# wenbowen123/catgrasp

Measured on NVIDIA H100. Metric: candidate grasps scored/sec, higher is better.
Workload: dtype f32 (128->1024 layer f16 x f16 single pass on wgmma, f32 accumulate; other layers bf16 hi/lo x3)

## Files before the change

catgrasp_b200/csrc/cg_trunk_tc.cu:

```cuda
#include <limits.h>
#include <stdlib.h>

#include <algorithm>

#include "cg_tc_ptx.cuh"
#include "cg_trunk_common.cuh"

namespace {
using namespace cg_trunk;
using namespace cg_ptx;

constexpr int NCW = 8;
constexpr int PROD_WARP = NCW;
constexpr int HELP_WARP = NCW + 1;
constexpr int NHELP = 3 * 32;
constexpr int NTC = (NCW + 4) * 32;
constexpr int NCHUNK = 8;
constexpr uint32_t PIECE = 16384;
__host__ __device__ constexpr int tile_points(int passes) { return passes == 1 ? 256 : 128; }
constexpr uint32_t W1_OFF = 0;
constexpr uint32_t W2_OFF = PIECE;
constexpr uint32_t X3_OFF = 3 * PIECE;
constexpr uint32_t X3_BYTES = 4 * PIECE;
constexpr uint32_t RING_OFF = X3_OFF + X3_BYTES;
constexpr uint32_t RING_BYTES = 6 * PIECE;
constexpr uint32_t KEYS_OFF = RING_OFF + RING_BYTES;
constexpr uint32_t KEYS_BYTES = 2 * 1024 * 4;
constexpr uint32_t MISC_OFF = KEYS_OFF + KEYS_BYTES;
constexpr int NSLOT_MAX = 6;
constexpr uint32_t IMG_W3B = NCHUNK * 2 * 2 * PIECE;
constexpr uint32_t IMG_W2 = 2 * PIECE, IMG_W1 = PIECE;
constexpr uint32_t IMG_W2_OFF = IMG_W3B, IMG_W1_OFF = IMG_W3B + IMG_W2;
constexpr uint32_t IMG_W3H_OFF = IMG_W1_OFF + IMG_W1;
constexpr uint32_t IMG_W3H = NCHUNK * 2 * PIECE;

struct Misc {
  float w0[6 * 64];
  float bias0[64];
  float bias1[64];
  float bias2[128];
  double pinv[12];
  double mean[6];
  double sden[6];
  float T3[12];
  unsigned long long full_bar[NSLOT_MAX];
  unsigned long long empty_bar[NSLOT_MAX];
  unsigned long long w_bar;
  unsigned long long cand_bar;
  unsigned long long front_bar;
  unsigned long long keys_bar[2];
};

constexpr size_t SMEM_BYTES = MISC_OFF + sizeof(Misc);
static_assert(SMEM_BYTES <= 232448, "exceeds the 227 KB per-CTA shared memory of sm_90");

#ifdef CG_EXPERIMENTS
enum { TL_START, TL_INPUT, TL_FRONT, TL_X3, TL_L3, TL_L3_WAIT, TL_RING, TL_NPHASE };
constexpr int TL_CTAS = 8, TL_REC = TL_NPHASE + 2;
__host__ __device__ constexpr int TL_STRIDE(int B) { return B >= TL_CTAS ? B / TL_CTAS : 1; }
#define TL_PARAM , unsigned long long *tl
#define TL_ARG(p) , p
#else
#define TL_PARAM
#define TL_ARG(p)
#endif

template <int PASSES>
__global__ void __launch_bounds__(NTC, 1) trunk_tc_kernel(const cg_trunk_args a TL_PARAM) {
  constexpr int TILE = tile_points(PASSES);
  constexpr int NBLK = TILE / 128;
  constexpr int NSLOT = PASSES == 3 ? 3 : 6;
  constexpr uint32_t SLOT_BYTES = PASSES == 3 ? 2 * PIECE : PIECE;
  static_assert(NSLOT * SLOT_BYTES == RING_BYTES, "ring");
  constexpr bool F16 = PASSES < 3;
  constexpr uint32_t X3_KB = TILE * 128;
  constexpr uint32_t X3_LO = 2 * X3_KB;
  static_assert((PASSES == 1 ? 2 : 4) * X3_KB == X3_BYTES, "X3 image");
  extern __shared__ __align__(1024) unsigned char smem[];
  if ((smem_u32(smem) & 1023u) != 0u) __trap();
  Misc &S = *reinterpret_cast<Misc *>(smem + MISC_OFF);
  uint32_t *keys = reinterpret_cast<uint32_t *>(smem + KEYS_OFF);
  const int tid = threadIdx.x, warp = __shfl_sync(0xffffffffu, tid >> 5, 0), lane = tid & 31;
  const int N = a.N;
  const int ntiles = (N + TILE - 1) / TILE;
  const long long T = (long long)a.B * ntiles;
  const int t_begin = (int)(blockIdx.x * T / gridDim.x);
  const int my_tiles = (int)((blockIdx.x + 1) * T / gridDim.x) - t_begin;
  const int b_first = t_begin / ntiles;
  const int ncand = (t_begin + my_tiles - 1) / ntiles - b_first + 1;
  const unsigned char *img = static_cast<const unsigned char *>(a.tc_img);
  const bool has_l1 = a.stage1_mode != 0;
  const uint32_t smem_s = smem_u32(smem);
  const uint32_t w1_s = smem_s + W1_OFF, w2_s = smem_s + W2_OFF, x3_s = smem_s + X3_OFF, ring_s = smem_s + RING_OFF;
  const uint32_t misc_s = smem_s + MISC_OFF;
  const uint32_t full_s = misc_s + (uint32_t)offsetof(Misc, full_bar), empty_s = misc_s + (uint32_t)offsetof(Misc, empty_bar);
  const uint32_t wbar_s = misc_s + (uint32_t)offsetof(Misc, w_bar);
  const uint32_t cand_s = misc_s + (uint32_t)offsetof(Misc, cand_bar), front_s = misc_s + (uint32_t)offsetof(Misc, front_bar);
  const uint32_t keys_s = misc_s + (uint32_t)offsetof(Misc, keys_bar);

  for (int i = tid; i < 6 * 64; i += NTC) S.w0[i] = a.l0.Wt[i];
  if (tid < 64) {
    S.bias0[tid] = a.l0.b[tid];
    S.bias1[tid] = (a.stage1_mode == 1) ? a.l1.b[tid] : 0.f;
  }
  if (tid < 128) S.bias2[tid] = a.l2.b[tid];
  if (a.in.x_direct == nullptr && tid < 6) {
    S.mean[tid] = a.in.mean ? a.in.mean[tid] : 0.0;
    S.sden[tid] = a.in.stdv ? 1.0 / (a.in.stdv[tid] + 1e-15) : 1.0;
  }
  if (tid == 0) {
    for (int i = 0; i < NSLOT; i++) {
      mbar_init(full_s + 8u * i, 1);
      mbar_init(empty_s + 8u * i, NCW);
    }
    mbar_init(wbar_s, 1);
    mbar_init(cand_s, NHELP);
    mbar_init(front_s, NCW * 32);
    mbar_init(keys_s, NCW * 32);
    mbar_init(keys_s + 8u, NCW * 32);
    mbar_init_fence();
  }
  __syncthreads();

  if (warp == PROD_WARP) {
    if (lane == 0) {
      mbar_expect_tx(wbar_s, IMG_W2 + (a.stage1_mode == 1 ? IMG_W1 : 0u));
      bulk_g2s(w2_s, img + IMG_W2_OFF, IMG_W2, wbar_s);
      if (a.stage1_mode == 1) bulk_g2s(w1_s, img + IMG_W1_OFF, IMG_W1, wbar_s);
      const unsigned char *w3src = img + (PASSES == 3 ? 0u : IMG_W3H_OFF);
      const int total = my_tiles * NCHUNK * 2;
      for (int gs = 0; gs < total; gs++) {
        const int s = gs % NSLOT;
        mbar_wait(empty_s + 8u * s, (((uint32_t)(gs / NSLOT)) & 1u) ^ 1u);
        mbar_expect_tx(full_s + 8u * s, SLOT_BYTES);
        bulk_g2s(ring_s + (uint32_t)s * SLOT_BYTES, w3src + (size_t)(gs % (NCHUNK * 2)) * SLOT_BYTES, SLOT_BYTES,
                 full_s + 8u * s);
      }
    }
    return;
  }

  if (warp >= HELP_WARP) {
    const int ht = tid - HELP_WARP * 32;
    for (int k = 0; k <= ncand; k++) {
      if (k < ncand) {
        const int b = b_first + k;
        constexpr int TU = (64 * 8 + NHELP - 1) / NHELP;
        uint32_t t64h[TU][4], t64l[TU][4];
        if (a.stage1_mode == 2) {
          const float *Tb = a.T64 + (size_t)b * 4096;
#pragma unroll
          for (int i = 0; i < TU; i++) {
            const int u = ht + NHELP * i;
            if (u < 512) {
              float v[8];
#pragma unroll
              for (int e = 0; e < 8; e++) v[e] = __ldg(Tb + (8 * (u >> 6) + e) * 64 + (u & 63));
#pragma unroll
              for (int e = 0; e < 4; e++) split_bf16x2(v[2 * e], v[2 * e + 1], t64h[i][e], t64l[i][e]);
            }
          }
        }
        double pinv[12];
        const bool do_pinv = a.in.x_direct == nullptr && ht == 0;
        if (do_pinv) pose_inverse(a.in.poses + (size_t)b * 16, pinv);
        const float t3 = (a.T3 && ht < 9) ? a.T3[b * 9 + ht] : 0.f;
        if (k > 0) mbar_wait(front_s, (uint32_t)(k - 1) & 1u);
        if (a.stage1_mode == 2) {
#pragma unroll
          for (int i = 0; i < TU; i++) {
            const int u = ht + NHELP * i;
            if (u < 512) {
              const uint32_t off = row_chunk_off(u & 63, u >> 6);
              *reinterpret_cast<uint4 *>(smem + W1_OFF + off) =
                  make_uint4(t64h[i][0], t64h[i][1], t64h[i][2], t64h[i][3]);
              *reinterpret_cast<uint4 *>(smem + W1_OFF + 8192 + off) =
                  make_uint4(t64l[i][0], t64l[i][1], t64l[i][2], t64l[i][3]);
            }
          }
          fence_proxy_async();
        }
        if (do_pinv) {
#pragma unroll
          for (int i = 0; i < 12; i++) S.pinv[i] = pinv[i];
        }
        if (ht < 9) S.T3[ht] = t3;
        mbar_arrive(cand_s);
      }
      if (k > 0) {
        const int kp = k - 1;
        mbar_wait(keys_s + 8u * (kp & 1), ((uint32_t)kp >> 1) & 1u);
        const uint32_t *kb = keys + (kp & 1) * 1024;
        uint32_t *g = a.gmax_keys + (size_t)(b_first + kp) * 1024;
        for (int ch = ht; ch < 1024; ch += NHELP) {
          float m = cg_key2f(kb[ch]) + __ldg(&a.l3.b[ch]);
          if (a.relu3) m = fmaxf(m, 0.f);
          atomicMax(&g[ch], cg_f2key(m));
        }
      }
    }
    return;
  }

  const int wg = warp >> 2, w4 = warp & 3, g = lane >> 2, q = lane & 3;
  float vmax = 0.f;
#ifdef CG_EXPERIMENTS
  const bool tl_on = tl != nullptr && blockIdx.x % TL_STRIDE(gridDim.x) == 0 &&
                     (int)(blockIdx.x / TL_STRIDE(gridDim.x)) < TL_CTAS;
  unsigned long long tl_sum[TL_NPHASE] = {}, tl_t0 = clock64(), tl_t = tl_t0, tl_s;
#define TL_MARK(phase)                   \
  do {                                   \
    const unsigned long long _t = clock64(); \
    tl_sum[phase] += _t - tl_t;          \
    tl_t = _t;                           \
  } while (0)
#define TL_SPAN_BEGIN() (tl_s = clock64())
#define TL_SPAN_END(phase) (tl_sum[phase] += clock64() - tl_s)
#else
#define TL_MARK(phase) ((void)0)
#define TL_SPAN_BEGIN() ((void)0)
#define TL_SPAN_END(phase) ((void)0)
#endif
  mbar_wait(wbar_s, 0u);

  auto fetch_id = [&](int b, int n) -> int {
    if (n >= N) n = N - 1;
    return (a.in.x_direct == nullptr && a.in.ids) ? __ldg(a.in.ids + (size_t)b * N + n) : n;
  };
  auto fetch_row = [&](int b, int id, double *r) {
    if (a.in.x_direct) {
      const float *xr = a.in.x_direct + ((size_t)b * N + id) * 6;
#pragma unroll
      for (int k = 0; k < 6; k++) r[k] = __ldg(xr + k);
    } else {
      const double *px = a.in.cloud_xyz + (size_t)id * 3;
      const double *pn = a.in.cloud_nrm + (size_t)id * 3;
#pragma unroll
      for (int k = 0; k < 3; k++) {
        r[k] = __ldg(px + k);
        r[3 + k] = __ldg(pn + k);
      }
    }
  };
  auto finish_row = [&](const double *r, float *v) {
    if (a.in.x_direct) {
#pragma unroll
      for (int k = 0; k < 6; k++) v[k] = (float)r[k];
    } else {
      const double x = r[0], y = r[1], z = r[2];
      const double nx = r[3], ny = r[4], nz = r[5];
      const double *R = S.pinv;
      double w[6];
      w[0] = R[0] * x + R[1] * y + R[2] * z + R[9];
      w[1] = R[3] * x + R[4] * y + R[5] * z + R[10];
      w[2] = R[6] * x + R[7] * y + R[8] * z + R[11];
      w[3] = R[0] * nx + R[1] * ny + R[2] * nz;
      w[4] = R[3] * nx + R[4] * ny + R[5] * nz;
      w[5] = R[6] * nx + R[7] * ny + R[8] * nz;
#pragma unroll
      for (int k = 0; k < 6; k++) v[k] = (float)((w[k] - S.mean[k]) * S.sden[k]);
    }
    if (a.T3) {
      const float x = v[0], y = v[1], z = v[2];
      v[0] = fmaf(z, S.T3[6], fmaf(y, S.T3[3], x * S.T3[0]));
      v[1] = fmaf(z, S.T3[7], fmaf(y, S.T3[4], x * S.T3[1]));
      v[2] = fmaf(z, S.T3[8], fmaf(y, S.T3[5], x * S.T3[2]));
    }
  };

  uint32_t gslot = 0;
  auto slot_of = [&](int c, int kb) { return (gslot + 2u * c + kb) % NSLOT; };
  auto phase_of = [&](int c, int kb) { return ((gslot + 2u * c + kb) / NSLOT) & 1u; };

  auto prow = [&](int blk) { return wg * (TILE / 2) + blk * 64 + w4 * 16 + g; };
  int ids[NBLK][2];
  {
    const int j = t_begin - b_first * ntiles;
#pragma unroll
    for (int blk = 0; blk < NBLK; blk++)
#pragma unroll
      for (int r = 0; r < 2; r++) ids[blk][r] = fetch_id(b_first, j * TILE + prow(blk) + 8 * r);
  }
  TL_MARK(TL_START);
  for (int it = 0; it < my_tiles; it++) {
    const int b = (t_begin + it) / ntiles, j = t_begin + it - b * ntiles, ci = b - b_first;
    const bool cand_first = it == 0 || j == 0, cand_last = it + 1 == my_tiles || j + 1 == ntiles;
    if (cand_first) mbar_wait(cand_s, (uint32_t)ci & 1u);
#pragma unroll 1
    for (int blk = 0; blk < NBLK; blk++) {
      const int p0 = j * TILE + prow(blk);
      float d64[32];
      {
        double r0[6], r1[6];
        fetch_row(b, blk == 0 ? ids[0][0] : ids[NBLK - 1][0], r0);
        fetch_row(b, blk == 0 ? ids[0][1] : ids[NBLK - 1][1], r1);
        float v0[6], v1[6];
        finish_row(r0, v0);
        finish_row(r1, v1);
        TL_MARK(TL_INPUT);
#pragma unroll
        for (int m = 0; m < 8; m++)
#pragma unroll
          for (int e = 0; e < 2; e++) {
            const int c = 8 * m + 2 * q + e;
            float o0 = S.bias0[c], o1 = o0;
#pragma unroll
            for (int k = 0; k < 6; k++) {
              const float w = S.w0[k * 64 + c];
              o0 = fmaf(v0[k], w, o0);
              o1 = fmaf(v1[k], w, o1);
            }
            d64[4 * m + e] = fmaxf(o0, 0.f);
            d64[4 * m + 2 + e] = fmaxf(o1, 0.f);
          }
      }
      uint32_t xh[4][4], xl[4][4];
      if (has_l1) {
        d_to_a<4, false>(d64, xh, xl);
        wg_fence_regs<16>(xh[0]);
        wg_fence_regs<16>(xl[0]);
        wg_fence_regs<32>(d64);
        wg_fence();
#pragma unroll
        for (int ks = 0; ks < 4; ks++) {
          const uint64_t bh = wg_desc(w1_s + 32u * ks), bl = wg_desc(w1_s + 8192u + 32u * ks);
          wg_m64n64<false>(d64, xl[ks], bh, ks > 0 ? 1u : 0u);
          wg_m64n64<false>(d64, xh[ks], bl, 1u);
          wg_m64n64<false>(d64, xh[ks], bh, 1u);
        }
        wg_commit();
        wg_wait<0>();
        wg_fence_regs<32>(d64);
        wg_fence_regs<16>(xh[0]);
        wg_fence_regs<16>(xl[0]);
#pragma unroll
        for (int i = 0; i < 32; i++) {
          if (a.stage1_mode == 1) d64[i] = fmaxf(d64[i] + S.bias1[8 * (i >> 2) + 2 * q + (i & 1)], 0.f);
        }
        if (a.pf_out) {
#pragma unroll
          for (int r = 0; r < 2; r++) {
            const int n = p0 + 8 * r;
            if (n < N) {
              float *dst = a.pf_out + ((size_t)b * N + n) * 64 + 2 * q;
#pragma unroll
              for (int m = 0; m < 8; m++)
                *reinterpret_cast<float2 *>(dst + 8 * m) = make_float2(d64[4 * m + 2 * r], d64[4 * m + 2 * r + 1]);
            }
          }
        }
      }
      if (cand_last && blk == NBLK - 1) mbar_arrive(front_s);
      float acc[64];
      d_to_a<4, false>(d64, xh, xl);
      wg_fence_regs<16>(xh[0]);
      wg_fence_regs<16>(xl[0]);
      wg_fence_regs<64>(acc);
      wg_fence();
#pragma unroll
      for (int ks = 0; ks < 4; ks++) {
        const uint64_t bh = wg_desc(w2_s + 32u * ks), bl = wg_desc(w2_s + PIECE + 32u * ks);
        wg_m64n128<false>(acc, xl[ks], bh, ks > 0 ? 1u : 0u);
        wg_m64n128<false>(acc, xh[ks], bl, 1u);
        wg_m64n128<false>(acc, xh[ks], bh, 1u);
      }
      wg_commit();
      wg_wait<0>();
      wg_fence_regs<64>(acc);
      wg_fence_regs<16>(xh[0]);
      wg_fence_regs<16>(xl[0]);
#pragma unroll
      for (int i = 0; i < 64; i++) acc[i] = fmaxf(acc[i] + S.bias2[8 * (i >> 2) + 2 * q + (i & 1)], 0.f);
      TL_MARK(TL_FRONT);
      if (blk == 0) asm volatile("bar.sync 1, 256;" ::: "memory");
#pragma unroll
      for (int r = 0; r < 2; r++) {
        const int pr = prow(blk) + 8 * r;
#pragma unroll
        for (int i = 0; i < 16; i++) {
          const float x0 = acc[4 * i + 2 * r], x1 = acc[4 * i + 2 * r + 1];
          const uint32_t off = X3_OFF + (uint32_t)(i >> 3) * X3_KB + row_chunk_off(pr, i & 7) + 4u * q;
          uint32_t h, l;
          if (PASSES == 1) {
            vmax = fmaxf(vmax, fmaxf(x0, x1));
            asm("cvt.rn.satfinite.f16x2.f32 %0, %1, %2;" : "=r"(h) : "f"(x1), "f"(x0));
          } else if (PASSES == 2) {
            vmax = fmaxf(vmax, fmaxf(x0, x1));
            split_f16x2(x0, x1, h, l);
          } else {
            split_bf16x2(x0, x1, h, l);
          }
          *reinterpret_cast<uint32_t *>(smem + off) = h;
          if (PASSES != 1) *reinterpret_cast<uint32_t *>(smem + off + X3_LO) = l;
        }
      }
    }
    fence_proxy_async();
    asm volatile("bar.sync 1, 256;" ::: "memory");
    TL_MARK(TL_X3);
    constexpr int NU = NCHUNK * NBLK, GROUP = PASSES == 1 ? 8 : (PASSES == 2 ? 4 : 1);
    constexpr bool EARLY_RELEASE = GROUP == 1;
    static_assert(GROUP == 1 || NSLOT >= 4, "a unit issued ahead needs the next chunk's slots as well");
    auto issue = [&](int u, float *d) {
      const int c = u / NBLK, hb = u % NBLK;
      if (hb == 0) {
        TL_SPAN_BEGIN();
        mbar_wait(full_s + 8u * slot_of(c, 0), phase_of(c, 0));
        mbar_wait(full_s + 8u * slot_of(c, 1), phase_of(c, 1));
        TL_SPAN_END(TL_RING);
      }
      wg_fence_regs<64>(d);
      wg_fence();
#pragma unroll
      for (int kb = 0; kb < 2; kb++) {
        const uint32_t ws = ring_s + slot_of(c, kb) * SLOT_BYTES + (uint32_t)wg * (PIECE / 2);
        const uint32_t xs = x3_s + (uint32_t)kb * X3_KB + (uint32_t)hb * PIECE;
#pragma unroll
        for (int ks = 0; ks < 4; ks++) {
          const uint32_t first = (kb | ks) ? 1u : 0u;
          const uint64_t aw = wg_desc(ws + 32u * ks), bx = wg_desc(xs + 32u * ks);
          if (PASSES == 3) {
            const uint64_t al = wg_desc(ws + PIECE + 32u * ks), bxl = wg_desc(xs + X3_LO + 32u * ks);
            wg_ss_m64n128<false>(d, aw, bxl, first);
            wg_ss_m64n128<false>(d, al, bx, 1u);
            wg_ss_m64n128<false>(d, aw, bx, 1u);
          } else if (PASSES == 2) {
            wg_ss_m64n128<true>(d, aw, wg_desc(xs + X3_LO + 32u * ks), first);
            wg_ss_m64n128<true>(d, aw, bx, 1u);
          } else {
            wg_ss_m64n128<true>(d, aw, bx, first);
          }
        }
        if (EARLY_RELEASE && kb == 0) wg_commit();
      }
      wg_commit();
      wg_fence_regs<64>(d);
    };
    uint32_t *kk = keys + (ci & 1) * 1024 + wg * 64 + w4 * 16 + g;
    auto reduce = [&](int u, const float *d) {
      const int c = u / NBLK, hb = u % NBLK;
      if (hb == NBLK - 1) {
        __syncwarp();
        if (lane == 0) {
          if (!EARLY_RELEASE) mbar_arrive(empty_s + 8u * slot_of(c, 0));
          mbar_arrive(empty_s + 8u * slot_of(c, 1));
        }
      }
#pragma unroll
      for (int r = 0; r < 2; r++) {
        float m = fmaxf(d[2 * r], d[2 * r + 1]);
#pragma unroll
        for (int i = 1; i < 16; i++) m = fmaxf(m, fmaxf(d[4 * i + 2 * r], d[4 * i + 2 * r + 1]));
        m = fmaxf(m, __shfl_xor_sync(0xffffffffu, m, 1));
        m = fmaxf(m, __shfl_xor_sync(0xffffffffu, m, 2));
        if (q == 0) {
          const uint32_t key = cg_f2key(m);
          uint32_t &slot = kk[128 * c + 8 * r];
          slot = (cand_first && hb == 0) ? key : max(slot, key);
        }
      }
    };
    {
      const int nt = t_begin + it + (it + 1 < my_tiles ? 1 : 0);
      const int nb = nt / ntiles, pn = (nt - nb * ntiles) * TILE;
#pragma unroll
      for (int blk = 0; blk < NBLK; blk++)
#pragma unroll
        for (int r = 0; r < 2; r++) ids[blk][r] = fetch_id(nb, pn + prow(blk) + 8 * r);
    }
#pragma unroll 1
    for (int u0 = 0; u0 < NU; u0 += GROUP) {
      float acc3[2][64];
      issue(u0, acc3[0]);
#pragma unroll
      for (int j = 0; j < GROUP; j++) {
        if (j + 1 < GROUP) issue(u0 + j + 1, acc3[(j + 1) & 1]);
        TL_SPAN_BEGIN();
        if (EARLY_RELEASE) {
          wg_wait<1>();
          __syncwarp();
          if (lane == 0) mbar_arrive(empty_s + 8u * slot_of((u0 + j) / NBLK, 0));
        }
        if (j + 1 < GROUP) wg_wait<1>();
        else wg_wait<0>();
        TL_SPAN_END(TL_L3_WAIT);
        wg_fence_regs<64>(acc3[j & 1]);
        reduce(u0 + j, acc3[j & 1]);
      }
    }
    gslot += 2u * NCHUNK;
    if (cand_last) mbar_arrive(keys_s + 8u * (ci & 1));
    TL_MARK(TL_L3);
  }
  if (F16 && vmax > 65504.f && a.ovf_flag) atomicOr(a.ovf_flag, 1u);
#ifdef CG_EXPERIMENTS
  if (tl_on && lane == 0) {
    unsigned long long *o = tl + ((size_t)(blockIdx.x / TL_STRIDE(gridDim.x)) * NCW + warp) * TL_REC;
#pragma unroll
    for (int p = 0; p < TL_NPHASE; p++) o[p] = tl_sum[p];
    o[TL_NPHASE] = (unsigned long long)my_tiles;
    o[TL_NPHASE + 1] = clock64() - tl_t0;
  }
#endif
#undef TL_MARK
#undef TL_SPAN_BEGIN
#undef TL_SPAN_END
}

}

size_t cg_tc_image_bytes() { return (size_t)IMG_W3H_OFF + IMG_W3H; }

int cg_tc_prepare(cg_ctx *ctx, const float *Wt3, const float *Wt2, const float *Wt1, void *dst_dev, int *f16_ok) {
  CG_CUDA(ctx, cudaFuncSetAttribute(trunk_tc_kernel<3>, cudaFuncAttributeMaxDynamicSharedMemorySize, (int)SMEM_BYTES));
  CG_CUDA(ctx, cudaFuncSetAttribute(trunk_tc_kernel<2>, cudaFuncAttributeMaxDynamicSharedMemorySize, (int)SMEM_BYTES));
  CG_CUDA(ctx, cudaFuncSetAttribute(trunk_tc_kernel<1>, cudaFuncAttributeMaxDynamicSharedMemorySize, (int)SMEM_BYTES));
  float wmax = 0.f;
  for (size_t i = 0; i < (size_t)128 * 1024; i++) wmax = fmaxf(wmax, fabsf(Wt3[i]));
  *f16_ok = (wmax < 65504.f) ? 1 : 0;
  std::vector<unsigned char> img(cg_tc_image_bytes(), 0);
  for (int ch = 0; ch < NCHUNK; ch++)
    for (int kb = 0; kb < 2; kb++) {
      unsigned char *hi = img.data() + (size_t)(ch * 2 + kb) * 2 * PIECE;
      cg_pack_bf16x2_block(Wt3, 1024, ch * 128, 128, kb * 64, hi, hi + PIECE);
    }
  cg_pack_bf16x2_block(Wt2, 128, 0, 128, 0, img.data() + IMG_W2_OFF, img.data() + IMG_W2_OFF + PIECE);
  if (Wt1) cg_pack_bf16x2_block(Wt1, 64, 0, 64, 0, img.data() + IMG_W1_OFF, img.data() + IMG_W1_OFF + 8192);
  for (int ch = 0; ch < NCHUNK; ch++)
    for (int r = 0; r < 128; r++)
      for (int k = 0; k < 128; k++) {
        const __half h = __float2half_rn(Wt3[(size_t)k * 1024 + ch * 128 + r]);
        unsigned short bits;
        memcpy(&bits, &h, 2);
        const size_t off = (size_t)IMG_W3H_OFF + (size_t)(ch * 2 + (k >> 6)) * PIECE + row_chunk_off(r, (k & 63) >> 3) +
                           (size_t)(k & 7) * 2;
        memcpy(img.data() + off, &bits, 2);
      }
  CG_CUDA(ctx, cudaMemcpyAsync(dst_dev, img.data(), img.size(), cudaMemcpyHostToDevice, ctx->stream));
  CG_CUDA(ctx, cudaStreamSynchronize(ctx->stream));
  return CG_OK;
}

int cg_trunk_launch_tc(cg_ctx *ctx, const cg_trunk_args &a) {
  CG_REQUIRE(ctx, a.B > 0 && a.N > 0, "trunk: B,N must be positive");
  CG_REQUIRE(ctx, a.tc_img != nullptr, "trunk: tensor-core weight image missing");
  const int passes = !a.tc_f16_ok || ctx->engine == 1 ? 3 : (ctx->engine == 2 ? 2 : 1);
  const int tp = tile_points(passes);
  const long long tiles = (long long)a.B * ((a.N + tp - 1) / tp);
  CG_REQUIRE(ctx, tiles <= INT_MAX, "trunk: too many tiles in one launch");
  const int grid = (int)std::min<long long>(ctx->num_sms, tiles);
#ifdef CG_EXPERIMENTS
  static const bool timeline = getenv("CG_TRUNK_TIMELINE") && atoi(getenv("CG_TRUNK_TIMELINE")) != 0;
  unsigned long long *tl = nullptr;
  const size_t tl_words = (size_t)TL_CTAS * NCW * TL_REC;
  if (timeline) {
    CG_CUDA(ctx, cudaMallocAsync(&tl, tl_words * 8, ctx->stream));
    CG_CUDA(ctx, cudaMemsetAsync(tl, 0, tl_words * 8, ctx->stream));
  }
#endif
  if (passes == 3) trunk_tc_kernel<3><<<grid, NTC, SMEM_BYTES, ctx->stream>>>(a TL_ARG(tl));
  else if (passes == 2) trunk_tc_kernel<2><<<grid, NTC, SMEM_BYTES, ctx->stream>>>(a TL_ARG(tl));
  else trunk_tc_kernel<1><<<grid, NTC, SMEM_BYTES, ctx->stream>>>(a TL_ARG(tl));
  CG_LAUNCH_CHECK(ctx);
#ifdef CG_EXPERIMENTS
  if (timeline) {
    std::vector<unsigned long long> h(tl_words);
    CG_CUDA(ctx, cudaMemcpyAsync(h.data(), tl, tl_words * 8, cudaMemcpyDeviceToHost, ctx->stream));
    CG_CUDA(ctx, cudaFreeAsync(tl, ctx->stream));
    CG_CUDA(ctx, cudaStreamSynchronize(ctx->stream));
    double sum[TL_NPHASE + 1] = {}, tiles = 0;
    int recs = 0;
    for (int r = 0; r < TL_CTAS * NCW; r++) {
      const unsigned long long *o = &h[(size_t)r * TL_REC];
      if (o[TL_NPHASE] == 0) continue;
      for (int p = 0; p < TL_NPHASE; p++) sum[p] += (double)o[p];
      sum[TL_NPHASE] += (double)o[TL_NPHASE + 1];
      tiles += (double)o[TL_NPHASE];
      recs++;
    }
    if (recs > 0) {
      const double p128 = tiles * (tp / 128);
      const double l3 = 128.0 * 128 * 1024 / 2048 * passes, l12 = 128.0 * 64 * (128 + (a.stage1_mode ? 64 : 0)) * 3 / 2048;
      const double tot = sum[TL_NPHASE] / p128;
      fprintf(stderr,
              "[trunk-timeline] passes=%d B=%d N=%d stage1=%d tile=%d tiles/CTA=%.0f warps=%d  clk/128 pts: start %.0f  "
              "input %.0f  front %.0f  x3 %.0f  l3 %.0f (wgmma-wait %.0f, ring-wait %.0f)  total %.0f  | tensor work "
              "%.0f clk/128 pts -> busy %.1f%%\n",
              passes, a.B, a.N, a.stage1_mode, tp, tiles / recs, recs, sum[TL_START] / p128, sum[TL_INPUT] / p128,
              sum[TL_FRONT] / p128, sum[TL_X3] / p128, sum[TL_L3] / p128, sum[TL_L3_WAIT] / p128, sum[TL_RING] / p128,
              tot, l3 + l12, 100.0 * (l3 + l12) / tot);
    }
  }
#endif
  return CG_OK;
}
```

Measured before the change: 521,800.

## Move per-point input gather and pose transform to helper warps via smem handoff

```diff
diff --git a/catgrasp_b200/csrc/cg_trunk_tc.cu b/catgrasp_b200/csrc/cg_trunk_tc.cu
--- a/catgrasp_b200/csrc/cg_trunk_tc.cu
+++ b/catgrasp_b200/csrc/cg_trunk_tc.cu
@@ -39,24 +39,25 @@
   float bias0[64];
   float bias1[64];
   float bias2[128];
-  double pinv[12];
   double mean[6];
   double sden[6];
-  float T3[12];
   unsigned long long full_bar[NSLOT_MAX];
   unsigned long long empty_bar[NSLOT_MAX];
   unsigned long long w_bar;
+  unsigned long long x0_full;
+  unsigned long long x0_empty;
   unsigned long long cand_bar;
   unsigned long long front_bar;
   unsigned long long keys_bar[2];
 };
-
-constexpr size_t SMEM_BYTES = MISC_OFF + sizeof(Misc);
-static_assert(SMEM_BYTES <= 232448, "exceeds the 227 KB per-CTA shared memory of sm_90");
+constexpr uint32_t X0_OFF = MISC_OFF + sizeof(Misc);
+__host__ __device__ constexpr size_t smem_bytes(int passes) { return X0_OFF + (size_t)tile_points(passes) * 6 * 4; }
+static_assert(smem_bytes(1) <= 232448 && smem_bytes(3) <= 232448, "exceeds the 227 KB per-CTA shared memory of sm_90");
 
 #ifdef CG_EXPERIMENTS
 enum { TL_START, TL_INPUT, TL_FRONT, TL_X3, TL_L3, TL_L3_WAIT, TL_RING, TL_NPHASE };
-constexpr int TL_CTAS = 8, TL_REC = TL_NPHASE + 2;
+enum { TH_BUILD, TH_EMPTY, TH_CAND, TH_FOLD, TH_NPHASE };
+constexpr int TL_CTAS = 8, TL_REC = TL_NPHASE + 2, TL_WARPS = NCW + 3;
 __host__ __device__ constexpr int TL_STRIDE(int B) { return B >= TL_CTAS ? B / TL_CTAS : 1; }
 #define TL_PARAM , unsigned long long *tl
 #define TL_ARG(p) , p
@@ -97,6 +98,9 @@
   const uint32_t wbar_s = misc_s + (uint32_t)offsetof(Misc, w_bar);
   const uint32_t cand_s = misc_s + (uint32_t)offsetof(Misc, cand_bar), front_s = misc_s + (uint32_t)offsetof(Misc, front_bar);
   const uint32_t keys_s = misc_s + (uint32_t)offsetof(Misc, keys_bar);
+  const uint32_t x0f_s = misc_s + (uint32_t)offsetof(Misc, x0_full), x0e_s = misc_s + (uint32_t)offsetof(Misc, x0_empty);
+  float *x0 = reinterpret_cast<float *>(smem + X0_OFF);
+  const bool t64_handoff = a.stage1_mode == 2;
 
   for (int i = tid; i < 6 * 64; i += NTC) S.w0[i] = a.l0.Wt[i];
   if (tid < 64) {
@@ -114,6 +118,8 @@
       mbar_init(empty_s + 8u * i, NCW);
     }
     mbar_init(wbar_s, 1);
+    mbar_init(x0f_s, NHELP);
+    mbar_init(x0e_s, NCW * 32);
     mbar_init(cand_s, NHELP);
     mbar_init(front_s, NCW * 32);
     mbar_init(keys_s, NCW * 32);
@@ -121,6 +127,34 @@
     mbar_init_fence();
   }
   __syncthreads();
+
+#ifdef CG_EXPERIMENTS
+  const bool tl_on = tl != nullptr && blockIdx.x % TL_STRIDE(gridDim.x) == 0 &&
+                     (int)(blockIdx.x / TL_STRIDE(gridDim.x)) < TL_CTAS;
+  unsigned long long tl_sum[TL_NPHASE] = {}, tl_t0 = clock64(), tl_t = tl_t0, tl_s;
+#define TL_MARK(phase)                   \
+  do {                                   \
+    const unsigned long long _t = clock64(); \
+    tl_sum[phase] += _t - tl_t;          \
+    tl_t = _t;                           \
+  } while (0)
+#define TL_SPAN_BEGIN() (tl_s = clock64())
+#define TL_SPAN_END(phase) (tl_sum[phase] += clock64() - tl_s)
+#define TL_WRITE(rec, tiles)                                                                              \
+  do {                                                                                                    \
+    if (tl_on && lane == 0) {                                                                             \
+      unsigned long long *o = tl + ((size_t)(blockIdx.x / TL_STRIDE(gridDim.x)) * TL_WARPS + (rec)) * TL_REC; \
+      for (int p = 0; p < TL_NPHASE; p++) o[p] = tl_sum[p];                                               \
+      o[TL_NPHASE] = (unsigned long long)(tiles);                                                         \
+      o[TL_NPHASE + 1] = clock64() - tl_t0;                                                               \
+    }                                                                                                     \
+  } while (0)
+#else
+#define TL_MARK(phase) ((void)0)
+#define TL_SPAN_BEGIN() ((void)0)
+#define TL_SPAN_END(phase) ((void)0)
+#define TL_WRITE(rec, tiles) ((void)0)
+#endif
 
   if (warp == PROD_WARP) {
     if (lane == 0) {
@@ -142,161 +176,179 @@
 
   if (warp >= HELP_WARP) {
     const int ht = tid - HELP_WARP * 32;
-    for (int k = 0; k <= ncand; k++) {
-      if (k < ncand) {
-        const int b = b_first + k;
+    constexpr int XR = (TILE + NHELP - 1) / NHELP;
+    const bool xd = a.in.x_direct != nullptr;
+    double pinv[12];
+    float t3[9] = {};
+    auto fetch_id = [&](int b, int n) -> int {
+      if (n >= N) n = N - 1;
+      return (!xd && a.in.ids) ? __ldg(a.in.ids + (size_t)b * N + n) : n;
+    };
+    auto fetch_row = [&](int b, int id, double *r) {
+      if (xd) {
+        const float *xr = a.in.x_direct + ((size_t)b * N + id) * 6;
+#pragma unroll
+        for (int k = 0; k < 6; k++) r[k] = __ldg(xr + k);
+      } else {
+        const double *px = a.in.cloud_xyz + (size_t)id * 3;
+        const double *pn = a.in.cloud_nrm + (size_t)id * 3;
+#pragma unroll
+        for (int k = 0; k < 3; k++) {
+          r[k] = __ldg(px + k);
+          r[3 + k] = __ldg(pn + k);
+        }
+      }
+    };
+    auto finish_row = [&](const double *r, float *v) {
+      if (xd) {
+#pragma unroll
+        for (int k = 0; k < 6; k++) v[k] = (float)r[k];
+      } else {
+        const double x = r[0], y = r[1], z = r[2];
+        const double nx = r[3], ny = r[4], nz = r[5];
+        const double *R = pinv;
+        double w[6];
+        w[0] = R[0] * x + R[1] * y + R[2] * z + R[9];
+        w[1] = R[3] * x + R[4] * y + R[5] * z + R[10];
+        w[2] = R[6] * x + R[7] * y + R[8] * z + R[11];
+        w[3] = R[0] * nx + R[1] * ny + R[2] * nz;
+        w[4] = R[3] * nx + R[4] * ny + R[5] * nz;
+        w[5] = R[6] * nx + R[7] * ny + R[8] * nz;
+#pragma unroll
+        for (int k = 0; k < 6; k++) v[k] = (float)((w[k] - S.mean[k]) * S.sden[k]);
+      }
+      if (a.T3) {
+        const float x = v[0], y = v[1], z = v[2];
+        v[0] = fmaf(z, t3[6], fmaf(y, t3[3], x * t3[0]));
+        v[1] = fmaf(z, t3[7], fmaf(y, t3[4], x * t3[1]));
+        v[2] = fmaf(z, t3[8], fmaf(y, t3[5], x * t3[2]));
+      }
+    };
+    auto fold = [&](int kp) {
+      mbar_wait(keys_s + 8u * (kp & 1), ((uint32_t)kp >> 1) & 1u);
+      const uint32_t *kb = keys + (kp & 1) * 1024;
+      uint32_t *g = a.gmax_keys + (size_t)(b_first + kp) * 1024;
+      for (int ch = ht; ch < 1024; ch += NHELP) {
+        float m = cg_key2f(kb[ch]) + __ldg(&a.l3.b[ch]);
+        if (a.relu3) m = fmaxf(m, 0.f);
+        atomicMax(&g[ch], cg_f2key(m));
+      }
+    };
+    int ids[XR];
+    auto load_ids = [&](int t) {
+      const int b = t / ntiles, j = t - b * ntiles;
+#pragma unroll
+      for (int i = 0; i < XR; i++)
+        if (ht + NHELP * i < TILE) ids[i] = fetch_id(b, j * TILE + ht + NHELP * i);
+    };
+    load_ids(t_begin);
+#pragma unroll 1
+    for (int it = 0; it < my_tiles; it++) {
+      const int b = (t_begin + it) / ntiles, j = t_begin + it - b * ntiles, ci = b - b_first;
+      const bool cand_first = it == 0 || j == 0;
+      if (cand_first && t64_handoff) {
         constexpr int TU = (64 * 8 + NHELP - 1) / NHELP;
         uint32_t t64h[TU][4], t64l[TU][4];
-        if (a.stage1_mode == 2) {
-          const float *Tb = a.T64 + (size_t)b * 4096;
-#pragma unroll
-          for (int i = 0; i < TU; i++) {
-            const int u = ht + NHELP * i;
-            if (u < 512) {
-              float v[8];
-#pragma unroll
-              for (int e = 0; e < 8; e++) v[e] = __ldg(Tb + (8 * (u >> 6) + e) * 64 + (u & 63));
-#pragma unroll
-              for (int e = 0; e < 4; e++) split_bf16x2(v[2 * e], v[2 * e + 1], t64h[i][e], t64l[i][e]);
-            }
+        const float *Tb = a.T64 + (size_t)b * 4096;
+#pragma unroll
+        for (int i = 0; i < TU; i++) {
+          const int u = ht + NHELP * i;
+          if (u < 512) {
+            float tv[8];
+#pragma unroll
+            for (int e = 0; e < 8; e++) tv[e] = __ldg(Tb + (8 * (u >> 6) + e) * 64 + (u & 63));
+#pragma unroll
+            for (int e = 0; e < 4; e++) split_bf16x2(tv[2 * e], tv[2 * e + 1], t64h[i][e], t64l[i][e]);
           }
         }
-        double pinv[12];
-        const bool do_pinv = a.in.x_direct == nullptr && ht == 0;
-        if (do_pinv) pose_inverse(a.in.poses + (size_t)b * 16, pinv);
-        const float t3 = (a.T3 && ht < 9) ? a.T3[b * 9 + ht] : 0.f;
-        if (k > 0) mbar_wait(front_s, (uint32_t)(k - 1) & 1u);
-        if (a.stage1_mode == 2) {
-#pragma unroll
-          for (int i = 0; i < TU; i++) {
-            const int u = ht + NHELP * i;
-            if (u < 512) {
-              const uint32_t off = row_chunk_off(u & 63, u >> 6);
-              *reinterpret_cast<uint4 *>(smem + W1_OFF + off) =
-                  make_uint4(t64h[i][0], t64h[i][1], t64h[i][2], t64h[i][3]);
-              *reinterpret_cast<uint4 *>(smem + W1_OFF + 8192 + off) =
-                  make_uint4(t64l[i][0], t64l[i][1], t64l[i][2], t64l[i][3]);
-            }
+        if (ci > 0) mbar_wait(front_s, (uint32_t)(ci - 1) & 1u);
+#pragma unroll
+        for (int i = 0; i < TU; i++) {
+          const int u = ht + NHELP * i;
+          if (u < 512) {
+            const uint32_t off = row_chunk_off(u & 63, u >> 6);
+            *reinterpret_cast<uint4 *>(smem + W1_OFF + off) =
+                make_uint4(t64h[i][0], t64h[i][1], t64h[i][2], t64h[i][3]);
+            *reinterpret_cast<uint4 *>(smem + W1_OFF + 8192 + off) =
+                make_uint4(t64l[i][0], t64l[i][1], t64l[i][2], t64l[i][3]);
           }
-          fence_proxy_async();
-        }
-        if (do_pinv) {
-#pragma unroll
-          for (int i = 0; i < 12; i++) S.pinv[i] = pinv[i];
-        }
-        if (ht < 9) S.T3[ht] = t3;
+        }
+        fence_proxy_async();
         mbar_arrive(cand_s);
-      }
-      if (k > 0) {
-        const int kp = k - 1;
-        mbar_wait(keys_s + 8u * (kp & 1), ((uint32_t)kp >> 1) & 1u);
-        const uint32_t *kb = keys + (kp & 1) * 1024;
-        uint32_t *g = a.gmax_keys + (size_t)(b_first + kp) * 1024;
-        for (int ch = ht; ch < 1024; ch += NHELP) {
-          float m = cg_key2f(kb[ch]) + __ldg(&a.l3.b[ch]);
-          if (a.relu3) m = fmaxf(m, 0.f);
-          atomicMax(&g[ch], cg_f2key(m));
-        }
-      }
-    }
+        TL_MARK(TH_CAND);
+      }
+      if (cand_first) {
+        if (!xd) pose_inverse(a.in.poses + (size_t)b * 16, pinv);
+        if (a.T3) {
+#pragma unroll
+          for (int e = 0; e < 9; e++) t3[e] = a.T3[b * 9 + e];
+        }
+      }
+      float v[XR][6];
+      {
+        double r[XR][6];
+#pragma unroll
+        for (int i = 0; i < XR; i++)
+          if (ht + NHELP * i < TILE) fetch_row(b, ids[i], r[i]);
+#pragma unroll
+        for (int i = 0; i < XR; i++)
+          if (ht + NHELP * i < TILE) finish_row(r[i], v[i]);
+      }
+      TL_MARK(TH_BUILD);
+      if (it > 0) mbar_wait(x0e_s, (uint32_t)(it - 1) & 1u);
+      TL_MARK(TH_EMPTY);
+#pragma unroll
+      for (int i = 0; i < XR; i++)
+        if (ht + NHELP * i < TILE) {
+          float2 *dst = reinterpret_cast<float2 *>(x0 + (ht + NHELP * i) * 6);
+          dst[0] = make_float2(v[i][0], v[i][1]);
+          dst[1] = make_float2(v[i][2], v[i][3]);
+          dst[2] = make_float2(v[i][4], v[i][5]);
+        }
+      mbar_arrive(x0f_s);
+      if (it + 1 < my_tiles) load_ids(t_begin + it + 1);
+      TL_MARK(TH_BUILD);
+      if (cand_first && ci > 0) {
+        fold(ci - 1);
+        TL_MARK(TH_FOLD);
+      }
+    }
+    fold(ncand - 1);
+    TL_MARK(TH_FOLD);
+    TL_WRITE(NCW + warp - HELP_WARP, my_tiles);
     return;
   }
 
   const int wg = warp >> 2, w4 = warp & 3, g = lane >> 2, q = lane & 3;
   float vmax = 0.f;
-#ifdef CG_EXPERIMENTS
-  const bool tl_on = tl != nullptr && blockIdx.x % TL_STRIDE(gridDim.x) == 0 &&
-                     (int)(blockIdx.x / TL_STRIDE(gridDim.x)) < TL_CTAS;
-  unsigned long long tl_sum[TL_NPHASE] = {}, tl_t0 = clock64(), tl_t = tl_t0, tl_s;
-#define TL_MARK(phase)                   \
-  do {                                   \
-    const unsigned long long _t = clock64(); \
-    tl_sum[phase] += _t - tl_t;          \
-    tl_t = _t;                           \
-  } while (0)
-#define TL_SPAN_BEGIN() (tl_s = clock64())
-#define TL_SPAN_END(phase) (tl_sum[phase] += clock64() - tl_s)
-#else
-#define TL_MARK(phase) ((void)0)
-#define TL_SPAN_BEGIN() ((void)0)
-#define TL_SPAN_END(phase) ((void)0)
-#endif
   mbar_wait(wbar_s, 0u);
-
-  auto fetch_id = [&](int b, int n) -> int {
-    if (n >= N) n = N - 1;
-    return (a.in.x_direct == nullptr && a.in.ids) ? __ldg(a.in.ids + (size_t)b * N + n) : n;
-  };
-  auto fetch_row = [&](int b, int id, double *r) {
-    if (a.in.x_direct) {
-      const float *xr = a.in.x_direct + ((size_t)b * N + id) * 6;
-#pragma unroll
-      for (int k = 0; k < 6; k++) r[k] = __ldg(xr + k);
-    } else {
-      const double *px = a.in.cloud_xyz + (size_t)id * 3;
-      const double *pn = a.in.cloud_nrm + (size_t)id * 3;
-#pragma unroll
-      for (int k = 0; k < 3; k++) {
-        r[k] = __ldg(px + k);
-        r[3 + k] = __ldg(pn + k);
-      }
-    }
-  };
-  auto finish_row = [&](const double *r, float *v) {
-    if (a.in.x_direct) {
-#pragma unroll
-      for (int k = 0; k < 6; k++) v[k] = (float)r[k];
-    } else {
-      const double x = r[0], y = r[1], z = r[2];
-      const double nx = r[3], ny = r[4], nz = r[5];
-      const double *R = S.pinv;
-      double w[6];
-      w[0] = R[0] * x + R[1] * y + R[2] * z + R[9];
-      w[1] = R[3] * x + R[4] * y + R[5] * z + R[10];
-      w[2] = R[6] * x + R[7] * y + R[8] * z + R[11];
-      w[3] = R[0] * nx + R[1] * ny + R[2] * nz;
-      w[4] = R[3] * nx + R[4] * ny + R[5] * nz;
-      w[5] = R[6] * nx + R[7] * ny + R[8] * nz;
-#pragma unroll
-      for (int k = 0; k < 6; k++) v[k] = (float)((w[k] - S.mean[k]) * S.sden[k]);
-    }
-    if (a.T3) {
-      const float x = v[0], y = v[1], z = v[2];
-      v[0] = fmaf(z, S.T3[6], fmaf(y, S.T3[3], x * S.T3[0]));
-      v[1] = fmaf(z, S.T3[7], fmaf(y, S.T3[4], x * S.T3[1]));
-      v[2] = fmaf(z, S.T3[8], fmaf(y, S.T3[5], x * S.T3[2]));
-    }
-  };
 
   uint32_t gslot = 0;
   auto slot_of = [&](int c, int kb) { return (gslot + 2u * c + kb) % NSLOT; };
   auto phase_of = [&](int c, int kb) { return ((gslot + 2u * c + kb) / NSLOT) & 1u; };
 
   auto prow = [&](int blk) { return wg * (TILE / 2) + blk * 64 + w4 * 16 + g; };
-  int ids[NBLK][2];
-  {
-    const int j = t_begin - b_first * ntiles;
-#pragma unroll
-    for (int blk = 0; blk < NBLK; blk++)
-#pragma unroll
-      for (int r = 0; r < 2; r++) ids[blk][r] = fetch_id(b_first, j * TILE + prow(blk) + 8 * r);
-  }
   TL_MARK(TL_START);
   for (int it = 0; it < my_tiles; it++) {
     const int b = (t_begin + it) / ntiles, j = t_begin + it - b * ntiles, ci = b - b_first;
     const bool cand_first = it == 0 || j == 0, cand_last = it + 1 == my_tiles || j + 1 == ntiles;
-    if (cand_first) mbar_wait(cand_s, (uint32_t)ci & 1u);
+    if (cand_first && t64_handoff) mbar_wait(cand_s, (uint32_t)ci & 1u);
+    mbar_wait(x0f_s, (uint32_t)it & 1u);
 #pragma unroll 1
     for (int blk = 0; blk < NBLK; blk++) {
       const int p0 = j * TILE + prow(blk);
       float d64[32];
       {
-        double r0[6], r1[6];
-        fetch_row(b, blk == 0 ? ids[0][0] : ids[NBLK - 1][0], r0);
-        fetch_row(b, blk == 0 ? ids[0][1] : ids[NBLK - 1][1], r1);
         float v0[6], v1[6];
-        finish_row(r0, v0);
-        finish_row(r1, v1);
+        const float2 *x0r = reinterpret_cast<const float2 *>(x0 + prow(blk) * 6);
+#pragma unroll
+        for (int k = 0; k < 3; k++) {
+          const float2 u0 = x0r[k], u1 = x0r[24 + k];
+          v0[2 * k] = u0.x;
+          v0[2 * k + 1] = u0.y;
+          v1[2 * k] = u1.x;
+          v1[2 * k + 1] = u1.y;
+        }
         TL_MARK(TL_INPUT);
 #pragma unroll
         for (int m = 0; m < 8; m++)
@@ -314,6 +366,7 @@
             d64[4 * m + 2 + e] = fmaxf(o1, 0.f);
           }
       }
+      if (blk == NBLK - 1) mbar_arrive(x0e_s);
       uint32_t xh[4][4], xl[4][4];
       if (has_l1) {
         d_to_a<4, false>(d64, xh, xl);
@@ -350,7 +403,7 @@
           }
         }
       }
-      if (cand_last && blk == NBLK - 1) mbar_arrive(front_s);
+      if (t64_handoff && cand_last && blk == NBLK - 1) mbar_arrive(front_s);
       float acc[64];
       d_to_a<4, false>(d64, xh, xl);
       wg_fence_regs<16>(xh[0]);
@@ -460,14 +513,6 @@
         }
       }
     };
-    {
-      const int nt = t_begin + it + (it + 1 < my_tiles ? 1 : 0);
-      const int nb = nt / ntiles, pn = (nt - nb * ntiles) * TILE;
-#pragma unroll
-      for (int blk = 0; blk < NBLK; blk++)
-#pragma unroll
-        for (int r = 0; r < 2; r++) ids[blk][r] = fetch_id(nb, pn + prow(blk) + 8 * r);
-    }
 #pragma unroll 1
     for (int u0 = 0; u0 < NU; u0 += GROUP) {
       float acc3[2][64];
@@ -493,18 +538,11 @@
     TL_MARK(TL_L3);
   }
   if (F16 && vmax > 65504.f && a.ovf_flag) atomicOr(a.ovf_flag, 1u);
-#ifdef CG_EXPERIMENTS
-  if (tl_on && lane == 0) {
-    unsigned long long *o = tl + ((size_t)(blockIdx.x / TL_STRIDE(gridDim.x)) * NCW + warp) * TL_REC;
-#pragma unroll
-    for (int p = 0; p < TL_NPHASE; p++) o[p] = tl_sum[p];
-    o[TL_NPHASE] = (unsigned long long)my_tiles;
-    o[TL_NPHASE + 1] = clock64() - tl_t0;
-  }
-#endif
+  TL_WRITE(warp, my_tiles);
 #undef TL_MARK
 #undef TL_SPAN_BEGIN
 #undef TL_SPAN_END
+#undef TL_WRITE
 }
 
 }
@@ -512,9 +550,9 @@
 size_t cg_tc_image_bytes() { return (size_t)IMG_W3H_OFF + IMG_W3H; }
 
 int cg_tc_prepare(cg_ctx *ctx, const float *Wt3, const float *Wt2, const float *Wt1, void *dst_dev, int *f16_ok) {
-  CG_CUDA(ctx, cudaFuncSetAttribute(trunk_tc_kernel<3>, cudaFuncAttributeMaxDynamicSharedMemorySize, (int)SMEM_BYTES));
-  CG_CUDA(ctx, cudaFuncSetAttribute(trunk_tc_kernel<2>, cudaFuncAttributeMaxDynamicSharedMemorySize, (int)SMEM_BYTES));
-  CG_CUDA(ctx, cudaFuncSetAttribute(trunk_tc_kernel<1>, cudaFuncAttributeMaxDynamicSharedMemorySize, (int)SMEM_BYTES));
+  CG_CUDA(ctx, cudaFuncSetAttribute(trunk_tc_kernel<3>, cudaFuncAttributeMaxDynamicSharedMemorySize, (int)smem_bytes(3)));
+  CG_CUDA(ctx, cudaFuncSetAttribute(trunk_tc_kernel<2>, cudaFuncAttributeMaxDynamicSharedMemorySize, (int)smem_bytes(2)));
+  CG_CUDA(ctx, cudaFuncSetAttribute(trunk_tc_kernel<1>, cudaFuncAttributeMaxDynamicSharedMemorySize, (int)smem_bytes(1)));
   float wmax = 0.f;
   for (size_t i = 0; i < (size_t)128 * 1024; i++) wmax = fmaxf(wmax, fabsf(Wt3[i]));
   *f16_ok = (wmax < 65504.f) ? 1 : 0;
@@ -552,15 +590,16 @@
 #ifdef CG_EXPERIMENTS
   static const bool timeline = getenv("CG_TRUNK_TIMELINE") && atoi(getenv("CG_TRUNK_TIMELINE")) != 0;
   unsigned long long *tl = nullptr;
-  const size_t tl_words = (size_t)TL_CTAS * NCW * TL_REC;
+  const size_t tl_words = (size_t)TL_CTAS * TL_WARPS * TL_REC;
   if (timeline) {
     CG_CUDA(ctx, cudaMallocAsync(&tl, tl_words * 8, ctx->stream));
     CG_CUDA(ctx, cudaMemsetAsync(tl, 0, tl_words * 8, ctx->stream));
   }
 #endif
-  if (passes == 3) trunk_tc_kernel<3><<<grid, NTC, SMEM_BYTES, ctx->stream>>>(a TL_ARG(tl));
-  else if (passes == 2) trunk_tc_kernel<2><<<grid, NTC, SMEM_BYTES, ctx->stream>>>(a TL_ARG(tl));
-  else trunk_tc_kernel<1><<<grid, NTC, SMEM_BYTES, ctx->stream>>>(a TL_ARG(tl));
+  const size_t smem = smem_bytes(passes);
+  if (passes == 3) trunk_tc_kernel<3><<<grid, NTC, smem, ctx->stream>>>(a TL_ARG(tl));
+  else if (passes == 2) trunk_tc_kernel<2><<<grid, NTC, smem, ctx->stream>>>(a TL_ARG(tl));
+  else trunk_tc_kernel<1><<<grid, NTC, smem, ctx->stream>>>(a TL_ARG(tl));
   CG_LAUNCH_CHECK(ctx);
 #ifdef CG_EXPERIMENTS
   if (timeline) {
@@ -568,27 +607,34 @@
     CG_CUDA(ctx, cudaMemcpyAsync(h.data(), tl, tl_words * 8, cudaMemcpyDeviceToHost, ctx->stream));
     CG_CUDA(ctx, cudaFreeAsync(tl, ctx->stream));
     CG_CUDA(ctx, cudaStreamSynchronize(ctx->stream));
-    double sum[TL_NPHASE + 1] = {}, tiles = 0;
+    double sum[TL_NPHASE + 1] = {}, tiles = 0, hsum[TH_NPHASE + 1] = {}, htiles = 0;
     int recs = 0;
-    for (int r = 0; r < TL_CTAS * NCW; r++) {
+    for (int r = 0; r < TL_CTAS * TL_WARPS; r++) {
       const unsigned long long *o = &h[(size_t)r * TL_REC];
       if (o[TL_NPHASE] == 0) continue;
-      for (int p = 0; p < TL_NPHASE; p++) sum[p] += (double)o[p];
-      sum[TL_NPHASE] += (double)o[TL_NPHASE + 1];
-      tiles += (double)o[TL_NPHASE];
-      recs++;
+      if (r % TL_WARPS < NCW) {
+        for (int p = 0; p < TL_NPHASE; p++) sum[p] += (double)o[p];
+        sum[TL_NPHASE] += (double)o[TL_NPHASE + 1];
+        tiles += (double)o[TL_NPHASE];
+        recs++;
+      } else {
+        for (int p = 0; p < TH_NPHASE; p++) hsum[p] += (double)o[p];
+        hsum[TH_NPHASE] += (double)o[TL_NPHASE + 1];
+        htiles += (double)o[TL_NPHASE];
+      }
     }
     if (recs > 0) {
-      const double p128 = tiles * (tp / 128);
+      const double p128 = tiles * (tp / 128), h128 = htiles * (tp / 128);
       const double l3 = 128.0 * 128 * 1024 / 2048 * passes, l12 = 128.0 * 64 * (128 + (a.stage1_mode ? 64 : 0)) * 3 / 2048;
       const double tot = sum[TL_NPHASE] / p128;
       fprintf(stderr,
               "[trunk-timeline] passes=%d B=%d N=%d stage1=%d tile=%d tiles/CTA=%.0f warps=%d  clk/128 pts: start %.0f  "
               "input %.0f  front %.0f  x3 %.0f  l3 %.0f (wgmma-wait %.0f, ring-wait %.0f)  total %.0f  | tensor work "
-              "%.0f clk/128 pts -> busy %.1f%%\n",
+              "%.0f clk/128 pts -> busy %.1f%%  | helpers: x0 build %.0f  x0-empty wait %.0f  t64 %.0f  fold %.0f\n",
               passes, a.B, a.N, a.stage1_mode, tp, tiles / recs, recs, sum[TL_START] / p128, sum[TL_INPUT] / p128,
               sum[TL_FRONT] / p128, sum[TL_X3] / p128, sum[TL_L3] / p128, sum[TL_L3_WAIT] / p128, sum[TL_RING] / p128,
-              tot, l3 + l12, 100.0 * (l3 + l12) / tot);
+              tot, l3 + l12, 100.0 * (l3 + l12) / tot, hsum[TH_BUILD] / h128, hsum[TH_EMPTY] / h128,
+              hsum[TH_CAND] / h128, hsum[TH_FOLD] / h128);
     }
   }
 #endif
```

Result: faster. 546,100, median of 6 (+4.7%).
